# Future-Power-Networks/MAPDN

Measured on AMD Instinct MI355X. Metric: env-steps/sec (whole node), case141 batch=4096, at 1/2/4/8 MI355X, higher is better.
Workload: dtype f64

## Files before the change

include/mapdn.h:

```cpp
#ifndef MAPDN_H
#define MAPDN_H

#include <stdint.h>

#ifdef __cplusplus
extern "C" {
#endif

#define MAPDN_OK 0
#define MAPDN_E_INVALID (-1)
#define MAPDN_E_TOPOLOGY (-2)
#define MAPDN_E_HIP (-3)
#define MAPDN_E_STATE (-4)
#define MAPDN_E_NOMEM (-5)
#define MAPDN_E_INTERNAL (-6)

#define MAPDN_N_INFO 11

enum { MAPDN_BARRIER_L1 = 0, MAPDN_BARRIER_L2 = 1, MAPDN_BARRIER_COURANT_BELTRAMI = 2,
       MAPDN_BARRIER_BOWL = 3, MAPDN_BARRIER_BUMP = 4 };

enum { MAPDN_SS_PV = 1, MAPDN_SS_DEMAND = 2, MAPDN_SS_REACTIVE = 4, MAPDN_SS_VM_PU = 8,
       MAPDN_SS_VA_DEGREE = 16, MAPDN_SS_ALL = 31 };

// ... 75 lines not shown
} mapdn_env_config;

typedef struct mapdn_dims_t {
  int32_t n_envs, n_bus, n_line, n_load, n_sgen, n_agents, n_actions, obs_size, state_size, n_info;
  int32_t is_radial;
  int32_t max_zone_size;
} mapdn_dims_t;

typedef struct mapdn_handle mapdn_handle;

const char* mapdn_last_error(const mapdn_handle* h);

int mapdn_create(const mapdn_netspec* net, const mapdn_env_config* cfg, int32_t n_envs,
                 int32_t device, mapdn_handle** out);
void mapdn_destroy(mapdn_handle* h);
int mapdn_dims(const mapdn_handle* h, mapdn_dims_t* out);

int mapdn_set_profiles(mapdn_handle* h, const double* pv, const double* load_p, const double* load_q,
                       int64_t n_rows, int32_t time_delta_min, int32_t days);

int mapdn_get_profile_stats(const mapdn_handle* h, double* stdv, double* smax);

int mapdn_reset(mapdn_handle* h, const int64_t* start_rows, int32_t add_noise, int32_t max_tries,
                void* stream);

int mapdn_step(mapdn_handle* h, const void* actions, int32_t actions_dtype, int32_t add_noise,
               double* reward, uint8_t* terminated, double* info, void* stream);

int mapdn_step_obs(mapdn_handle* h, const void* actions, int32_t actions_dtype, int32_t add_noise,
                   double* reward, uint8_t* terminated, double* info, void* obs, int32_t obs_dtype, void* stream);

int mapdn_get_obs(mapdn_handle* h, void* obs, int32_t dtype, void* stream);
int mapdn_get_state(mapdn_handle* h, void* state, int32_t dtype, void* stream);

int mapdn_get_results(mapdn_handle* h, double* vm_pu, double* va_degree, double* p_mw, double* q_mvar,
                      double* pl_mw, double* sgen_p, double* sgen_q, void* stream);
int mapdn_get_loads(mapdn_handle* h, double* load_p, double* load_q, void* stream);

int mapdn_get_start_rows(mapdn_handle* h, int64_t* start_rows, void* stream);

int mapdn_get_auto_reset_mask(mapdn_handle* h, uint8_t* mask, void* stream);

int mapdn_get_returns(mapdn_handle* h, double* returns, void* stream);

int mapdn_solve_only(mapdn_handle* h, const double* p_load, const double* q_load, const double* p_sgen,
                     const double* q_sgen, double* vm_pu, double* va_degree, int32_t* iterations,
                     uint8_t* converged, void* stream);

int mapdn_get_ybus_dense(const mapdn_handle* h, double* ybus_re_im);
int mapdn_get_obs_index(const mapdn_handle* h, int32_t* kind, int32_t* index);

int mapdn_get_schedule(const mapdn_handle* h, int32_t n_waves, int32_t* n_rows, int32_t* rows, int32_t* parent);

int mapdn_get_nr_geometry(const mapdn_handle* h, int32_t* out20);

int mapdn_get_flat_factors(const mapdn_handle* h, double* factors, int32_t* bus_of_pos);

int mapdn_get_sparse_program(const mapdn_handle* h, int32_t sub_lanes, int32_t* dims, int32_t* ops, int32_t* order, int32_t* slots_ij);

int mapdn_dense_solve(const double* a, const double* b, double* x, int32_t n, int32_t batch, void* stream);

int mapdn_policy_forward(const float* obs, const float* hid_in, const float* w1, const float* b1, const float* ln_g,
                         const float* ln_b, const float* w_ih, const float* w_hh, const float* b_ih, const float* b_hh,
                         const float* w2, const float* b2, float* means, float* hid_out, int32_t rows, int32_t n_agents,
                         int32_t obs_dim, int32_t id_dim, float ln_eps, void* stream);

int mapdn_policy_forward_train(const float* obs, const float* hid_in, const float* w1, const float* b1, const float* ln_g,
                               const float* ln_b, const float* w_ih, const float* w_hh, const float* b_ih, const float* b_hh,
                               const float* w2, const float* b2, float* means, float* hid_out, float* x1_out, int32_t rows,
                               int32_t n_agents, int32_t obs_dim, int32_t id_dim, float ln_eps, void* stream);
int64_t mapdn_policy_backward_scratch_floats(int64_t rows);
int mapdn_policy_backward(const float* dmeans, const float* x1, const float* hid_in, const float* ln_g, const float* ln_b, float ln_eps,
                          const float* w_ih, const float* w_hh, const float* b_ih, const float* b_hh, const float* w2, float* dx1,
                          float* dgates, float* xn, float* small, float* scratch, int64_t rows, void* stream);

int mapdn_policy_forward_fits(int32_t obs_dim, int32_t id_dim);

int mapdn_layernorm64_forward(const float* x, const float* gamma, const float* beta, float* y, float* mean, float* rstd,
                              int64_t rows, float eps, int32_t relu, void* stream);
int mapdn_layernorm64_backward_blocks(int64_t rows);
int mapdn_layernorm64_backward(const float* dy, const float* x, const float* gamma, const float* beta, const float* mean,
                               const float* rstd, float* dx, float* dgamma, float* dbeta, float* partial, int64_t rows,
                               int32_t relu, void* stream);
int mapdn_layernorm64_bc_forward(const float* base, const float* per_n, int32_t n, const float* gamma, const float* beta, float* y,
                                 float* mean, float* rstd, int64_t rows, float eps, int32_t relu, void* stream);
int mapdn_layernorm64_bc_backward(const float* dy, const float* base, const float* per_n, int32_t n, const float* gamma, const float* beta,
                                  const float* mean, const float* rstd, float* dx, float* dgamma, float* dbeta, float* partial,
                                  int64_t rows, int32_t relu, void* stream);
int mapdn_relu_dot64_forward(const float* pre, const float* w, float bias, float* v, int64_t rows, void* stream);
int mapdn_relu_dot64_backward(const float* dv, const float* pre, const float* w, float* dpre, float* dw, float* db, float* partial,
                              int64_t rows, void* stream);

int mapdn_critic_head_forward(const float* x, const float* per_n, int32_t n, const float* gamma, const float* beta, float eps,
                              const float* w2, const float* b2, const float* w3, const float* b3, float* v, int64_t rows, void* stream);
int64_t mapdn_critic_head_scratch_floats(int64_t rows, int32_t n, int32_t formed);
int mapdn_critic_head_backward(const float* dv, const float* x, const float* per_n, int32_t n, const float* gamma, const float* beta,
                               float eps, const float* w2, const float* b2, const float* w3, const float* b3, float* dx, float* grads,
                               float* scratch, int64_t rows, int32_t param_grads, void* stream);
int mapdn_critic_head_mse(const float* ret, const float* wrow, const float* scale, const float* x, const float* per_n, int32_t n,
                          const float* gamma, const float* beta, float eps, const float* w2, const float* b2, const float* w3,
                          const float* b3, float* dx, float* grads, float* scratch, int64_t rows, void* stream);
int mapdn_critic_head_backward_dot(const float* dv, const float* x, const float* per_n, int32_t n, const float* gamma, const float* beta,
                                   float eps, const float* w2, const float* b2, const float* w3, const float* b3, const float* dot_w,
                                   float* dact, int64_t rows, void* stream);

int mapdn_explore_actions(const float* mean, const float* eps, const float* avail, float stdv, int32_t tanh_bound, double action_scale,
// ... 20 lines not shown
```

mapdn_amd/_lib.py:

```python
from __future__ import annotations

import ctypes as C
import os

import numpy as np

from .netspec import NetSpec

_HERE = os.path.dirname(os.path.abspath(__file__))
LIB_PATH = os.path.join(_HERE, "libmapdn_hip.so")

N_INFO = 11
INFO_KEYS = (
    "percentage_of_v_out_of_control", "percentage_of_lower_than_lower_v",
    "percentage_of_higher_than_upper_v", "totally_controllable_ratio",
    "average_voltage_deviation", "average_voltage", "max_voltage_drop_deviation",
    "max_voltage_rise_deviation", "total_line_loss", "q_loss", "destroy",
)
BARRIER_IDS = dict(l1=0, l2=1, courant_beltrami=2, bowl=3, bump=4)
SS_BITS = dict(pv=1, demand=2, reactive=4, vm_pu=8, va_degree=16)
F32, F64 = 0, 1

EXPORTS = (
    "mapdn_last_error", "mapdn_create", "mapdn_destroy", "mapdn_dims", "mapdn_set_profiles", "mapdn_reset",
    "mapdn_step", "mapdn_get_start_rows", "mapdn_get_returns", "mapdn_get_obs", "mapdn_get_state", "mapdn_get_results", "mapdn_get_loads",
    "mapdn_solve_only", "mapdn_get_ybus_dense", "mapdn_get_obs_index", "mapdn_get_schedule", "mapdn_get_flat_factors", "mapdn_stats", "mapdn_nr_timing",
    "mapdn_nr_time_ms", "mapdn_get_auto_reset_mask", "mapdn_dense_solve", "mapdn_step_obs", "mapdn_get_sparse_program", "mapdn_policy_forward",
    "mapdn_policy_forward_fits", "mapdn_layernorm64_forward", "mapdn_layernorm64_backward", "mapdn_layernorm64_backward_blocks",
    "mapdn_get_nr_geometry", "mapdn_debug_stream", "mapdn_build_info", "mapdn_layernorm64_bc_forward", "mapdn_layernorm64_bc_backward", "mapdn_relu_dot64_forward", "mapdn_relu_dot64_backward",
    "mapdn_critic_head_forward", "mapdn_critic_head_scratch_floats", "mapdn_critic_head_backward", "mapdn_critic_head_backward_dot", "mapdn_critic_head_mse", "mapdn_get_profile_stats",
    "mapdn_explore_actions", "mapdn_rollout_stats", "mapdn_copy_segments",
    "mapdn_policy_forward_train", "mapdn_policy_backward", "mapdn_policy_backward_scratch_floats",
)

_pd = C.POINTER(C.c_double)
_pi = C.POINTER(C.c_int32)
_pu8 = C.POINTER(C.c_uint8)


class CNetSpec(C.Structure):
    _fields_ = [
        ("n_bus", C.c_int32), ("bus_vn_kv", _pd), ("bus_zone", _pi),
        ("n_line", C.c_int32), ("line_from_bus", _pi), ("line_to_bus", _pi),
        ("line_r_ohm_per_km", _pd), ("line_x_ohm_per_km", _pd), ("line_c_nf_per_km", _pd),
        ("line_g_us_per_km", _pd), ("line_length_km", _pd), ("line_parallel", _pi), ("line_in_service", _pu8),
        ("n_branch_pu", C.c_int32), ("br_from_bus", _pi), ("br_to_bus", _pi), ("br_r_pu", _pd), ("br_x_pu", _pd),
        ("br_b_pu", _pd), ("br_ratio", _pd), ("br_shift_deg", _pd),
        ("n_shunt", C.c_int32), ("shunt_bus", _pi), ("shunt_p_mw", _pd), ("shunt_q_mvar", _pd),
        ("n_load", C.c_int32), ("load_bus", _pi),
        ("n_sgen", C.c_int32), ("sgen_bus", _pi), ("sgen_zone", _pi),
        ("ext_grid_bus", C.c_int32), ("ext_grid_vm_pu", C.c_double), ("sn_mva", C.c_double), ("f_hz", C.c_double),
        ("br_g_pu", _pd), ("load_scaling", _pd), ("sgen_scaling", _pd), ("bus_alias", _pi),
    ]


class CEnvConfig(C.Structure):
    _fields_ = [
        ("barrier_type", C.c_int32), ("voltage_weight", C.c_double), ("q_weight", C.c_double),
        ("line_weight", C.c_double), ("use_line_weight", C.c_int32), ("use_q_weight", C.c_int32),
        ("v_lower", C.c_double), ("v_upper", C.c_double), ("episode_limit", C.c_int32),
        ("action_low", C.c_double), ("action_high", C.c_double), ("reset_action", C.c_int32),
        ("state_space", C.c_int32), ("seed", C.c_uint64), ("env_id_offset", C.c_int64), ("auto_reset", C.c_int32),
        ("nr_solver", C.c_int32), ("nr_waves", C.c_int32), ("nr_lanes", C.c_int32), ("nr_lean", C.c_int32),
        ("nr_h_lds", C.c_int32), ("nr_g_lds", C.c_int32), ("nr_rec_lds", C.c_int32), ("nr_flat_lds", C.c_int32), ("nr_line_lds", C.c_int32),
        ("nr_mm_pass", C.c_int32), ("sp_lanes", C.c_int32), ("inject_full", C.c_int32),
        ("nr_check_dx", C.c_double), ("nr_check_quad", C.c_double), ("debug_geometry", C.c_int32),
        ("tolerance_mva", C.c_double), ("tolerance_is_pu", C.c_int32), ("nr_init", C.c_int32),
        ("fuse_inject", C.c_int32), ("overlap_advance", C.c_int32), ("xcd_map", C.c_int32),
    ]


TUNING_INT = ("nr_solver", "nr_waves", "nr_lanes", "nr_lean", "nr_h_lds", "nr_g_lds", "nr_rec_lds", "nr_flat_lds", "nr_line_lds",
              "nr_mm_pass", "sp_lanes", "inject_full", "debug_geometry", "tolerance_is_pu", "nr_init", "fuse_inject", "overlap_advance", "xcd_map")
TUNING_F64 = ("nr_check_dx", "nr_check_quad", "tolerance_mva")
NR_SOLVERS = dict(auto=0, tree=0, sparse=1, dense=2)
GEOMETRY_KEYS = ("solver", "waves", "lanes", "lean", "rows", "h_lds", "g_lds", "rec_lds", "flat_lds", "line_lds", "mm_pass",
                 "lds_bytes", "workgroups", "resident_per_cu", "rounds", "model_ns", "fuse_inject", "n_fused_buses", "n_nodes", "reserved")


class CDims(C.Structure):
    _fields_ = [(k, C.c_int32) for k in (
        "n_envs", "n_bus", "n_line", "n_load", "n_sgen", "n_agents", "n_actions", "obs_size", "state_size",
        "n_info", "is_radial", "max_zone_size")]


# ... 17 lines not shown
    global _lib
    if _lib is not None:
        return _lib
    import torch
    if "MAPDN_LIB_PATH" not in os.environ:
        from . import build as _build
        try:
            is_stale = _build.stale()
        except OSError:
            is_stale = not os.path.exists(LIB_PATH)
            if not is_stale:
                import warnings
                warnings.warn(f"mapdn_amd/csrc is not readable: {LIB_PATH} is loaded without the source-hash check", RuntimeWarning, stacklevel=2)
        if is_stale:
            try:
                _build.build_locked()
            except Exception as exc:
                raise ImportError(
                    f"{LIB_PATH} is missing or was built from other sources than mapdn_amd/csrc (hash {_build.library_hash()} vs "
                    f"{_safe_source_hash(_build)}) and could not be rebuilt ({exc}); build it with `python -m mapdn_amd.build` "
                    "(hipcc --offload-arch=gfx950); there is no CPU fallback") from exc
    lib = C.CDLL(os.environ.get("MAPDN_LIB_PATH", LIB_PATH))
    if "MAPDN_LIB_PATH" in os.environ:
        for name in EXPORTS:
            if not hasattr(lib, name):
                def _missing(*a, _n=name, **k):
                    raise AttributeError(f"{os.environ['MAPDN_LIB_PATH']} does not export {_n}")
                lib.__dict__[name] = _missing
    vp = C.c_void_p
    lib.mapdn_last_error.restype = C.c_char_p
    lib.mapdn_last_error.argtypes = [vp]
    lib.mapdn_build_info.restype = C.c_char_p
    lib.mapdn_build_info.argtypes = []
    lib.mapdn_create.argtypes = [C.POINTER(CNetSpec), C.POINTER(CEnvConfig), C.c_int32, C.c_int32, C.POINTER(vp)]
    lib.mapdn_destroy.argtypes = [vp]
    lib.mapdn_destroy.restype = None
    lib.mapdn_dims.argtypes = [vp, C.POINTER(CDims)]
    lib.mapdn_set_profiles.argtypes = [vp, _pd, _pd, _pd, C.c_int64, C.c_int32, C.c_int32]
    lib.mapdn_get_profile_stats.argtypes = [vp, _pd, _pd]
    lib.mapdn_reset.argtypes = [vp, vp, C.c_int32, C.c_int32, vp]
    lib.mapdn_step.argtypes = [vp, vp, C.c_int32, C.c_int32, vp, vp, vp, vp]
    lib.mapdn_step_obs.argtypes = [vp, vp, C.c_int32, C.c_int32, vp, vp, vp, vp, C.c_int32, vp]
    lib.mapdn_get_start_rows.argtypes = [vp, vp, vp]
    lib.mapdn_get_returns.argtypes = [vp, vp, vp]
    lib.mapdn_get_auto_reset_mask.argtypes = [vp, vp, vp]
    lib.mapdn_get_obs.argtypes = [vp, vp, C.c_int32, vp]
    lib.mapdn_get_state.argtypes = [vp, vp, C.c_int32, vp]
    lib.mapdn_get_results.argtypes = [vp] + [vp] * 7 + [vp]
    lib.mapdn_get_loads.argtypes = [vp, vp, vp, vp]
    lib.mapdn_solve_only.argtypes = [vp] + [vp] * 8 + [vp]
    lib.mapdn_get_ybus_dense.argtypes = [vp, _pd]
    lib.mapdn_get_obs_index.argtypes = [vp, _pi, _pi]
    lib.mapdn_get_schedule.argtypes = [vp, C.c_int32, _pi, _pi, _pi]
    lib.mapdn_get_flat_factors.argtypes = [vp, _pd, _pi]
    lib.mapdn_get_nr_geometry.argtypes = [vp, _pi]
    lib.mapdn_debug_stream.argtypes = [vp, vp, C.c_int32, C.c_int32, C.c_int32, vp]
    lib.mapdn_get_sparse_program.argtypes = [vp, C.c_int32, _pi, _pi, _pi, _pi]
    lib.mapdn_policy_forward.argtypes = [vp] * 14 + [C.c_int32] * 4 + [C.c_float, vp]
    lib.mapdn_policy_forward_fits.argtypes = [C.c_int32, C.c_int32]
    lib.mapdn_policy_forward_train.argtypes = [vp] * 15 + [C.c_int32] * 4 + [C.c_float, vp]
    lib.mapdn_policy_backward_scratch_floats.argtypes = [C.c_int64]
    lib.mapdn_policy_backward_scratch_floats.restype = C.c_int64
    lib.mapdn_policy_backward.argtypes = [vp] * 5 + [C.c_float] + [vp] * 10 + [C.c_int64, vp]
    lib.mapdn_layernorm64_forward.argtypes = [vp] * 6 + [C.c_int64, C.c_float, C.c_int32, vp]
    lib.mapdn_layernorm64_backward_blocks.argtypes = [C.c_int64]
    lib.mapdn_layernorm64_backward.argtypes = [vp] * 10 + [C.c_int64, C.c_int32, vp]
    lib.mapdn_layernorm64_bc_forward.argtypes = [vp, vp, C.c_int32] + [vp] * 5 + [C.c_int64, C.c_float, C.c_int32, vp]
    lib.mapdn_layernorm64_bc_backward.argtypes = [vp, vp, vp, C.c_int32] + [vp] * 8 + [C.c_int64, C.c_int32, vp]
    lib.mapdn_relu_dot64_forward.argtypes = [vp, vp, C.c_float, vp, C.c_int64, vp]
    lib.mapdn_relu_dot64_backward.argtypes = [vp] * 7 + [C.c_int64, vp]
    lib.mapdn_critic_head_forward.argtypes = [vp, vp, C.c_int32, vp, vp, C.c_float] + [vp] * 5 + [C.c_int64, vp]
    lib.mapdn_critic_head_scratch_floats.argtypes = [C.c_int64, C.c_int32, C.c_int32]
    lib.mapdn_critic_head_scratch_floats.restype = C.c_int64
    lib.mapdn_critic_head_backward.argtypes = [vp, vp, vp, C.c_int32, vp, vp, C.c_float] + [vp] * 7 + [C.c_int64, C.c_int32, vp]
    lib.mapdn_explore_actions.argtypes = [vp, vp, vp, C.c_float, C.c_int32, C.c_double, C.c_double, vp, vp, vp, C.c_int64, vp]
    lib.mapdn_rollout_stats.argtypes = [vp, vp, vp, vp, vp, vp, C.c_int32, vp]
    lib.mapdn_copy_segments.argtypes = [C.POINTER(vp), C.POINTER(vp), C.POINTER(C.c_int64), C.c_int32, vp]
    lib.mapdn_critic_head_mse.argtypes = [vp] * 5 + [C.c_int32, vp, vp, C.c_float] + [vp] * 7 + [C.c_int64, vp]
    lib.mapdn_critic_head_backward_dot.argtypes = [vp, vp, vp, C.c_int32, vp, vp, C.c_float] + [vp] * 6 + [C.c_int64, vp]
    lib.mapdn_dense_solve.argtypes = [vp, vp, vp, C.c_int32, C.c_int32, vp]
    lib.mapdn_stats.argtypes = [vp, C.POINTER(C.c_int64), C.POINTER(C.c_double), C.POINTER(C.c_int32), vp]
    lib.mapdn_nr_timing.argtypes = [vp, C.c_int32]
    lib.mapdn_nr_time_ms.argtypes = [vp, C.POINTER(C.c_double), C.POINTER(C.c_int64)]
    for name in EXPORTS:
        if name not in ("mapdn_last_error", "mapdn_destroy", "mapdn_build_info"):
            getattr(lib, name).restype = C.c_int
    _lib = lib
    return lib


def check(rc, handle=None):
    if rc != 0:
        msg = load().mapdn_last_error(handle)
        raise MapdnError(rc, msg.decode() if msg else "?")


def _p(a, typ):
    return a.ctypes.data_as(typ) if a.size else C.cast(None, typ)


def make_cnetspec(net: NetSpec):
    keep = net
    s = CNetSpec()
    s.n_bus = net.n_bus
    s.bus_vn_kv = _p(net.bus_vn_kv, _pd)
    s.bus_zone = _p(net.bus_zone, _pi)
# ... 78 lines not shown
```

mapdn_amd/csrc/capi.hip:

```cpp
#include <hip/hip_runtime.h>

#include <algorithm>
#include <cmath>
#include <cstdio>
#include <cstdlib>
#include <cstring>
#include <string>
#include <vector>

#include "kernels.hpp"
#include "colstats.hpp"
#include "plan.hpp"

using namespace mapdn;

struct mapdn_handle {
  Plan plan;
  Schedule sched;
  SparseProg sprog;
  int solver = 0;
  int sp_lanes = 0;
  mapdn_env_config cfg;
  Dev d;
  int device = 0;
// ... 797 lines not shown

int mapdn_get_ybus_dense(const mapdn_handle* h, double* out) try {
  if (!h || !out) return MAPDN_E_INVALID;
  const Plan& P = h->plan;
  for (size_t i = 0; i < P.ybus.size(); ++i) { out[2 * i] = P.ybus[i].real(); out[2 * i + 1] = P.ybus[i].imag(); }
  return MAPDN_OK;
} MAPDN_CATCH(h)

int mapdn_get_obs_index(const mapdn_handle* h, int32_t* kind, int32_t* index) try {
  if (!h || !kind || !index) return MAPDN_E_INVALID;
  std::memcpy(kind, h->plan.obs_kind.data(), h->plan.obs_kind.size() * sizeof(int32_t));
  std::memcpy(index, h->plan.obs_idx.data(), h->plan.obs_idx.size() * sizeof(int32_t));
  return MAPDN_OK;
} MAPDN_CATCH(h)

int mapdn_get_nr_geometry(const mapdn_handle* h, int32_t* out) try {
  if (!h || !out) return MAPDN_E_INVALID;
  const mapdn_handle::Geo& g = h->geo;
  const bool fuse_possible = h->solver == 0 && !h->cfg.auto_reset && !knob_int(h->cfg.inject_full, "MAPDN_INJECT_FULL") &&
                             knob_tri(h->cfg.fuse_inject, "MAPDN_FUSE_INJECT") != 2;
  const int32_t v[20] = {h->solver, g.W, g.L, g.lean, g.rows, g.h_lds, g.g_lds, g.rec_lds, g.flat_lds, g.line_lds, g.mm_pass,
                         (int32_t)h->lds_bytes, (int32_t)g.wgs, g.resident, g.rounds, (int32_t)std::min(g.model_ns, 2.0e9),
                         (h->host_only ? fuse_possible : h->fuse_inject) ? 1 : 0, (int32_t)h->plan.fused_obus.size(), h->plan.nb, 0};
  std::memcpy(out, v, sizeof(v));
  if (h->solver == 1) out[2] = h->sp_lanes;
  return MAPDN_OK;
} MAPDN_CATCH(h)

int mapdn_get_flat_factors(const mapdn_handle* h, double* factors, int32_t* bus_of_pos) try {
  if (!h || !factors) return MAPDN_E_INVALID;
  if (!h->plan.radial) return MAPDN_E_TOPOLOGY;
  Schedule S;
  build_schedule(h->plan, 1, S);
  const int n = h->plan.n;
  for (int r = 0; r < S.R; ++r) {
    const StepRec& T = S.steps[(size_t)r];
    if (T.flags & S_LIVE) std::memcpy(factors + (size_t)(T.kp & 0xffffu) * FLAT_N, &S.flat[(size_t)r * FLAT_N], FLAT_N * sizeof(double));
  }
  if (bus_of_pos) std::memcpy(bus_of_pos, h->plan.bus_of_pos.data(), (size_t)(n + 1) * sizeof(int32_t));
  return MAPDN_OK;
} MAPDN_CATCH(h)

int mapdn_get_schedule(const mapdn_handle* h, int32_t W, int32_t* n_rows, int32_t* rows, int32_t* parent) try {
  if (!h || !n_rows || W < 1 || W > 16) return MAPDN_E_INVALID;
  if (!h->plan.radial) return MAPDN_E_TOPOLOGY;
  Schedule S;
  build_schedule(h->plan, W, S);
  *n_rows = S.R;
  if (rows) for (size_t i = 0; i < S.steps.size(); ++i) rows[i] = (S.steps[i].flags & S_LIVE) ? (int32_t)(S.steps[i].kp & 0xffffu) : -1;
  if (parent) std::memcpy(parent, h->plan.par.data(), h->plan.par.size() * sizeof(int32_t));
  return MAPDN_OK;
} MAPDN_CATCH(h)

int mapdn_get_sparse_program(const mapdn_handle* h, int32_t S, int32_t* dims, int32_t* ops, int32_t* order, int32_t* slots_ij) try {
  if (!h || !dims || S < 1 || S > 64) return MAPDN_E_INVALID;
  SparseProg G;
  sparse_program(h->plan, S, G);
  dims[0] = G.n_blocks; dims[1] = G.n_fill; dims[2] = G.n_phases; dims[3] = G.rows_per_sub; dims[4] = G.max_nnz;
  dims[5] = (int32_t)(G.slots_ij.size() / 3);
  if (ops) std::memcpy(ops, G.ops.data(), G.ops.size() * sizeof(SpOp));
  if (order) std::memcpy(order, G.order.data(), G.order.size() * sizeof(int32_t));
  if (slots_ij) std::memcpy(slots_ij, G.slots_ij.data(), G.slots_ij.size() * sizeof(int32_t));
  return MAPDN_OK;
} MAPDN_CATCH(h)

int mapdn_dense_solve(const double* a, const double* b, double* x, int32_t n, int32_t batch, void* stream) try {
  if (!a || !b || !x) return MAPDN_E_INVALID;
  const int rc = dense_solve_debug(a, b, x, n, batch, (hipStream_t)stream);
  return rc == 0 ? MAPDN_OK : (rc == -1 ? MAPDN_E_INVALID : MAPDN_E_HIP);
} MAPDN_CATCH(nullptr)

int mapdn_stats(mapdn_handle* h, int64_t* reset_failures, double* mean_iters, int32_t* max_iters, void* stream) try {
  if (!h) return MAPDN_E_INVALID;
  NEEDDEV(h);
  HIPCHK(h, hipSetDevice(h->device));
  hipStream_t st = (hipStream_t)stream;
  launch_stats(h->d, h->stats_dev, st);
  long long host[4];
  HIPCHK(h, hipMemcpyAsync(host, h->stats_dev, sizeof(host), hipMemcpyDeviceToHost, st));
  HIPCHK(h, hipStreamSynchronize(st));
  if (reset_failures) *reset_failures = host[0];
  if (mean_iters) *mean_iters = host[2] ? (double)host[1] / (double)host[2] : 0.0;
  if (max_iters) *max_iters = (int32_t)host[3];
  return MAPDN_OK;
} MAPDN_CATCH(h)

int mapdn_nr_timing(mapdn_handle* h, int32_t enable) try {
  if (!h) return MAPDN_E_INVALID;
  h->timing = enable != 0;
  return MAPDN_OK;
} MAPDN_CATCH(h)

int mapdn_nr_time_ms(mapdn_handle* h, double* total_ms, int64_t* launches) try {
  if (!h) return MAPDN_E_INVALID;
  NEEDDEV(h);
  HIPCHK(h, hipSetDevice(h->device));
  double ms = h->acc_ms; int64_t n = h->acc_launches;
  for (size_t i = 0; i + 1 < h->ev_used; i += 2) {
    HIPCHK(h, hipEventSynchronize(h->ev[i + 1]));
    float t = 0.f;
    HIPCHK(h, hipEventElapsedTime(&t, h->ev[i], h->ev[i + 1]));
    ms += t; n += 1;
  }
  h->ev_used = 0; h->acc_ms = 0.0; h->acc_launches = 0;
  if (total_ms) *total_ms = ms;
  if (launches) *launches = n;
// ... 5 lines not shown
```

mapdn_amd/csrc/nr_tree.hpp:

```cpp
#pragma once
#include <hip/hip_runtime.h>
#include <stdint.h>

#include <type_traits>

#include "kernels.hpp"
#include "nr_common.hpp"

namespace mapdn {


#ifdef MAPDN_NR_STAMPS
static __device__ unsigned long long g_stamps[4096];
#define STAMP(id) do { if (stamp_on && ns < 4095) g_stamps[++ns] = ((unsigned long long)(id) << 48) | (__builtin_readcyclecounter() & 0xffffffffffffull); } while (0)
#ifdef MAPDN_NR_STAMPS_FINE
#define STAMP2(id) STAMP(id)
#else
#define STAMP2(id) do { } while (0)
#endif
#else
#define STAMP(id) do { } while (0)
#define STAMP2(id) do { } while (0)
#endif

// ... 491 lines not shown
            if (nch > 2) {
              auto gather = [&](unsigned slot) { const d2 a = cs[((size_t)slot * 4 + 3) * L]; aR0 += a.x; aR1 += a.y; };
              gather((chs >> 20) & 1023u);
              const unsigned cptr = clist_ptr(fl, slots, chs);
#pragma unroll 1
              for (int j = 3; j < nch; ++j) gather((unsigned)s_clist[cptr + j - 3]);
            }
          }
        }
        const double r0 = Fp - aR0, r1 = Fq - aR1;
        const double h0 = i0 * r0 + i1 * r1, h1 = i2 * r0 + i3 * r1;
        const double t0 = ap_i * h0 + ap_r * h1, t1 = ap_i * h1 - ap_r * h0;
        cR0 = t0; cR1 = t1;
        if (flu & SU_W_ANY) cs[((size_t)(slots & 1023u) * 4 + 3) * L] = d2{t0, t1};
        SCHED_FENCE();
        const unsigned k = kp & 0xffffu;
        if (HL) sH[(size_t)k * L] = d2{h0, h1}; else bst2(d2{h0, h1}, rs, voE + k * bb, sF_H);
        STAMP2(232);
        if (W > 1) lds_barrier();
        STAMP(102);
        ++r;
      }
    }
  };
  double dxm = 0.0;
  auto apply_update = [&](double y0, double y1, d2 vk, unsigned k, bool live) {
    dxm = fmax(dxm, live ? fmax(fabs(y0), fabs(y1)) : 0.0);
    double s, c;
    const double dth = -y0;
    sincos_small(dth, &s, &c);
    if (__any(live && !(fabs(dth) <= 0.5))) sincos_mid(dth, &s, &c);
    sV[(size_t)k * L] = done ? vk : nr_rotate(vk, s, c, y1);
  };
  constexpr int UPN = NR_UPDATE_GROUP;
  auto apply_update3 = [&](const d2 (&xx)[UPN], const d2 (&vv)[UPN], const unsigned (&kk)[UPN], const bool (&lv)[UPN]) {
    double s[UPN], c[UPN];
    bool big = false;
#pragma unroll
    for (int i = 0; i < UPN; ++i) {
      dxm = fmax(dxm, lv[i] ? fmax(fabs(xx[i].x), fabs(xx[i].y)) : 0.0);
      sincos_small(-xx[i].x, &s[i], &c[i]);
      big = big | (lv[i] & !(fabs(xx[i].x) <= 0.5));
    }
    if (__any(big)) {
#pragma unroll
      for (int i = 0; i < UPN; ++i) if (__any(lv[i] && !(fabs(xx[i].x) <= 0.5))) sincos_mid(-xx[i].x, &s[i], &c[i]);
    }
#pragma unroll
    for (int i = 0; i < UPN; ++i) sV[(size_t)kk[i] * L] = done ? vv[i] : nr_rotate(vv[i], s[i], c[i], xx[i].y);
  };
  auto bwd_xprop = [&](auto src) {
    constexpr int SRC = decltype(src)::value;
    constexpr bool gG = (SRC == 1) && !GL;
    u32x4 ixq[4]; d2 g01q[4], g23q[4];
    auto load_g = [&](int row, const u32x4& ixr, int slot) {
      if constexpr (SRC == 0) {
        if (flatL) { const char* p = flatT + (unsigned)row * FB; g01q[slot] = *(const d2*)(p + FL_G0 * 8); g23q[slot] = *(const d2*)(p + FL_G2 * 8); }
        else { const unsigned sf = row_s(row, FB); g01q[slot] = bld2(rsF, voF + FL_G0 * 8u, sf); g23q[slot] = bld2(rsF, voF + FL_G2 * 8u, sf); }
      } else if constexpr (gG) {
        const unsigned voN = voE + (ixr.w & 0xffffu) * bb;
        g01q[slot] = bld2(rs, voN, sF_G01); g23q[slot] = bld2(rs, voN, sF_G23);
      }
    };
    constexpr int KP = gG ? KR : 0;
    u32x4 ixs[KP > 0 ? KP : 1];
    static_for<KP>([&](auto ic) { constexpr int i = decltype(ic)::value; ixs[i] = load_ix(i); });
    ixq[0] = load_ix(R - 1); ixq[1] = load_ix(max(R - 2, 0)); ixq[2] = load_ix(max(R - 3, 0));
    load_g(R - 1, ixq[0], 0); load_g(max(R - 2, 0), ixq[1], 1);
    int r = R - 1;
    while (r >= KP) {
#pragma unroll
      for (int u = 0; u < 4; ++u) {
        if (r < KP) break;
        const uint32_t fl = ixq[u % 4].x, kp = ixq[u % 4].w;
        const unsigned k = kp & 0xffffu, p = kp >> 16;
        const d2 q = sH[(size_t)p * L];
        const d2 hh = sH[(size_t)k * L];
        d2 g01, g23;
        if constexpr (SRC == 1 && GL) { g01 = sG[(size_t)(2 * k) * L]; g23 = sG[(size_t)(2 * k + 1) * L]; }
        ixq[(u + 3) % 4] = load_ix(max(r - 3, KP));
        load_g(max(r - 2, KP), ixq[(u + 2) % 4], (u + 2) % 4);
        SCHED_FENCE();
        STAMP2(240);
        if constexpr (SRC == 0 || gG) { g01 = g01q[u % 4]; g23 = g23q[u % 4]; }
        const bool cout = (fl & S_CARRY_OUT) != 0;
        const double p0 = cout ? x0 : q.x, p1 = cout ? x1 : q.y;
        const double y0 = hh.x - (g01.x * p0 + g01.y * p1);
        const double y1 = hh.y - (g23.x * p0 + g23.y * p1);
        x0 = y0; x1 = y1;
        sH[(size_t)k * L] = d2{y0, y1};
        STAMP2(242);
        if (W > 1) lds_barrier();
        STAMP(110 + SRC);
        --r;
      }
    }
    static_for_down<KP>([&](auto ic) {
      constexpr int i = decltype(ic)::value;
      {
        const uint32_t fl = ixs[i].x, kp = ixs[i].w;
        const unsigned k = kp & 0xffffu, p = kp >> 16;
        const d2 q = sH[(size_t)p * L];
        const d2 hh = sH[(size_t)k * L];
        SCHED_FENCE();
        const bool cout = (fl & S_CARRY_OUT) != 0;
        const double p0 = cout ? x0 : q.x, p1 = cout ? x1 : q.y;
        const double G0 = a_get(Ga[i][0], Ga[i][1]), G1 = a_get(Ga[i][2], Ga[i][3]), G2 = a_get(Ga[i][4], Ga[i][5]), G3 = a_get(Ga[i][6], Ga[i][7]);
        const double y0 = hh.x - (G0 * p0 + G1 * p1);
        const double y1 = hh.y - (G2 * p0 + G3 * p1);
        x0 = y0; x1 = y1;
        sH[(size_t)k * L] = d2{y0, y1};
        if (W > 1) lds_barrier();
        STAMP(110 + SRC);
      }
    });
    for (unsigned kb = t; kb < n; kb += (unsigned)UPN * Wt) {
      unsigned kk[UPN]; d2 xx[UPN], vv[UPN]; bool lv[UPN];
#pragma unroll
      for (int i = 0; i < UPN; ++i) {
        const unsigned kx = kb + (unsigned)i * Wt;
        lv[i] = kx < n; kk[i] = lv[i] ? kx : n + 1u;
        xx[i] = sH[(size_t)kk[i] * L]; vv[i] = sV[(size_t)kk[i] * L];
      }
      apply_update3(xx, vv, kk, lv);
      STAMP(30);
    }
  };
  auto mismatch_pass = [&]() {
    const __amdgpu_buffer_rsrc_t rsP = __builtin_amdgcn_make_buffer_rsrc(const_cast<StepRec*>(d.mm_recs), 0, d.mm_recs_bytes, 0x00020000);
    const int NPs = d.mm_np;
    const unsigned voP = t * (unsigned)NPs * TB;
    {
      u32x4 ixn = bldu4(rsP, voP, 0u); d2 ypn = bld2(rsP, voP + 48u, 0u);
      for (int j = 0; j < NPs; ++j) {
        const u32x4 ix = ixn; const d2 ypk = ypn;
        const unsigned sn = row_s(min(j + 1, NPs - 1), TB);
        ixn = bldu4(rsP, voP, sn); ypn = bld2(rsP, voP + 48u, sn);
        const unsigned k = ix.w & 0xffffu, pp = ix.w >> 16;
        const d2 vk = sV[(size_t)k * L], vp = sV[(size_t)pp * L];
        const double ek = vk.x, fk = vk.y, ep = vp.x, fp = vp.y, gpk = ypk.x, bpk = ypk.y;
        const double ur = gpk * ek - bpk * fk, ui = gpk * fk + bpk * ek;
        const double apk_r = ep * ur + fp * ui, apk_i = fp * ur - ep * ui;
        sH[(size_t)k * L] = d2{apk_r, apk_i};
      }
    }
    STAMP(31);
    if (W > 1) lds_barrier();
    {
      const unsigned voSb = d.sb_off + e * 16u;
      auto cl = [&](int j) { return row_s(min(j, NPs - 1), TB); };
      u32x4 ixA = bldu4(rsP, voP, 0u), ixB = bldu4(rsP, voP, cl(1));
      d2 ykkN = bld2(rsP, voP + 16u, 0u), ykpN = bld2(rsP, voP + 32u, 0u), cksN = bld2(rsP, voP + 64u, 0u);
      d2 sbN = bld2(rs, voSb + (ixA.w & 0xffffu) * pb, 0u);
      for (int j = 0; j < NPs; ++j) {
        const u32x4 ix = ixA;
        const d2 ykk = ykkN, ykp = ykpN, cks = cksN, sb = sbN;
        const unsigned k = ix.w & 0xffffu, pp = ix.w >> 16;
        const int nch = (int)((ix.x >> 8) & 255u);
        const d2 vk = sV[(size_t)k * L], vp = sV[(size_t)pp * L];
        const d2 a0 = sH[(size_t)(ix.y & 0xffffu) * L], a1 = sH[(size_t)(ix.y >> 16) * L], a2 = sH[(size_t)(ix.z & 0xffffu) * L];
        {
          const unsigned s1 = cl(j + 1);
          ykkN = bld2(rsP, voP + 16u, s1); ykpN = bld2(rsP, voP + 32u, s1); cksN = bld2(rsP, voP + 64u, s1);
          sbN = bld2(rs, voSb + (ixB.w & 0xffffu) * pb, 0u);
          ixA = ixB; ixB = bldu4(rsP, voP, cl(j + 2));
        }
        const double gkk = ykk.x, bkk = ykk.y, gkp = ykp.x, bkp = ykp.y;
        const double ek = vk.x, fk = vk.y, ep = vp.x, fp = vp.y;
// ... 168 lines not shown
```

mapdn_amd/csrc/plan.cpp:

```cpp
#include "plan.hpp"

#include <algorithm>
#include <cmath>
#include <map>

namespace mapdn {

namespace {

struct PiBranch {
  int32_t f, t;
  cplx yff, yft, ytf, ytt;
};

PiBranch pi_from_line(const mapdn_netspec& net, int l) {
  const int f = net.line_from_bus[l], t = net.line_to_bus[l];
  const double vn = net.bus_vn_kv[f];
  const double base_r = vn * vn / net.sn_mva;
  const double len = net.line_length_km[l];
  const double par = (double)net.line_parallel[l];
  const double r = net.line_r_ohm_per_km[l] * len / base_r / par;
  const double x = net.line_x_ohm_per_km[l] * len / base_r / par;
  const double b = 2.0 * net.f_hz * M_PI * net.line_c_nf_per_km[l] * 1e-9 * base_r * len * par;
  const double g = net.line_g_us_per_km[l] * 1e-6 * base_r * len * par;
// ... 510 lines not shown
    }
    S.n_xslots = std::max(next, 1);
  }
  const uint32_t c_zero = (uint32_t)S.n_cslots, c_trash = c_zero + 1; S.n_cslots += 2;
  const uint32_t x_zero = (uint32_t)S.n_xslots, x_trash = x_zero + 1; S.n_xslots += 2;
  S.step_of_node.assign(n + 1, -1);
  for (int w = 0; w < W; ++w)
    for (int r = 0; r < R; ++r) {
      StepRec& T = S.steps[(size_t)w * R + r];
      const int k = rows[r][w];
      T = StepRec{};
      T.kp = (uint32_t)(n + 1) | ((uint32_t)n << 16);
      T.slots = c_trash | (x_trash << 10) | (x_zero << 20);
      T.chs = c_zero | (c_zero << 10) | (c_zero << 20);
      T.ykk[0] = 1.0; T.ykk[1] = -1.0; T.ykp[0] = -1.0; T.ykp[1] = 1.0; T.ypk[0] = -1.0; T.ypk[1] = 1.0;
      if (k < 0) continue;
      S.step_of_node[k] = w * R + r;
      const double* c = &P.yc[(size_t)k * 8];
      T.ykk[0] = c[0]; T.ykk[1] = c[1]; T.ykp[0] = c[2]; T.ykp[1] = c[3]; T.ypk[0] = c[4]; T.ypk[1] = c[5];
      T.cks[0] = c[6]; T.cks[1] = c[7];
      const int p = P.par[k];
      T.kp = (uint32_t)k | ((uint32_t)p << 16);
      uint32_t f = S_LIVE, os = c_trash, xsl = x_trash, pxs = x_zero;
      if (p == n) f |= S_PARENT_ROOT;
      else if (carry_out[k]) f |= S_CARRY_OUT;
      else { f |= S_SCRATCH_OUT; os = (uint32_t)oslot[k]; pxs = (uint32_t)xslot[p]; }
      std::vector<int> kids;
      const int cc = chain_child(k);
      if (cc >= 0) { if (carry_out[cc]) f |= S_CARRY_IN; else kids.push_back(oslot[cc]); }
      for (int ch : children[k]) if (ch != cc) kids.push_back(oslot[ch]);
      uint32_t ch3[3] = {c_zero, c_zero, c_zero};
      for (size_t j = 0; j < kids.size() && j < 3; ++j) ch3[j] = (uint32_t)kids[j];
      const uint32_t cptr = (uint32_t)S.clist.size();
      for (size_t j = 3; j < kids.size(); ++j) S.clist.push_back(kids[j]);
      if (xslot[k] >= 0) { f |= S_X_OUT; xsl = (uint32_t)xslot[k]; }
      T.slots = os | (xsl << 10) | (pxs << 20) | (((cptr >> 8) & 3u) << 30);
      T.chs = ch3[0] | (ch3[1] << 10) | (ch3[2] << 20) | (((cptr >> 10) & 3u) << 30);
      T.flags = f | ((uint32_t)std::min<size_t>(kids.size(), 255) << 16) | ((cptr & 255u) << 24);
    }
  for (int w0 = 0; w0 < W; w0 += Sw)
    for (int r = 0; r < R; ++r) {
      uint32_t gmax = 0, any = 0;
      for (int w = w0; w < w0 + Sw; ++w) {
        const StepRec& T = S.steps[(size_t)w * R + r];
        if (!(T.flags & S_LIVE)) continue;
        gmax = std::max(gmax, std::min<uint32_t>((T.flags >> 16) & 255u, 3u));
        if (T.flags & S_SCRATCH_OUT) any |= SU_W_ANY;
        if (T.flags & S_X_OUT) any |= SU_XW_ANY;
        if ((T.flags & S_SCRATCH_OUT)) any |= SU_XR_ANY;
        if (T.cks[0] != 0.0 || T.cks[1] != 0.0) any |= SU_SLACK_ANY;
      }
      for (int w = w0; w < w0 + Sw; ++w) S.steps[(size_t)w * R + r].flags |= (gmax << SU_GMAX_SHIFT) | any;
    }
  if (S.clist.empty()) S.clist.push_back(0);
  S.mm_ptr.assign(1, 0); S.mm_child.clear();
  for (int k = 0; k < n; ++k) {
    const int cc = chain_child(k);
    if (cc >= 0) S.mm_child.push_back(cc);
    for (int ch : children[k]) if (ch != cc) S.mm_child.push_back(ch);
    S.mm_ptr.push_back((int32_t)S.mm_child.size());
  }
  if (S.mm_child.empty()) S.mm_child.push_back(0);
  S.mm_np = (n + W - 1) / W;
  S.mm_recs.assign((size_t)W * S.mm_np, StepRec{});
  for (int w = 0; w < W; ++w)
    for (int j = 0; j < S.mm_np; ++j) {
      StepRec& T = S.mm_recs[(size_t)w * S.mm_np + j];
      const int kx = w + j * W;
      const bool live = kx < n;
      const int k = live ? kx : n - 1;
      const int c_lo = S.mm_ptr[k], nch = live ? S.mm_ptr[k + 1] - c_lo : 0;
      auto child = [&](int q) { return (uint32_t)(q < nch ? S.mm_child[c_lo + q] : n + 1); };
      T.flags = (live ? 1u : 0u) | ((uint32_t)std::min(nch, 255) << 8);
      T.slots = child(0) | (child(1) << 16);
      T.chs = child(2);
      T.kp = (uint32_t)k | ((uint32_t)P.par[k] << 16);
      const double* c = &P.yc[(size_t)k * 8];
      T.ykk[0] = c[0]; T.ykk[1] = c[1]; T.ykp[0] = c[2]; T.ykp[1] = c[3]; T.ypk[0] = c[4]; T.ypk[1] = c[5]; T.cks[0] = c[6]; T.cks[1] = c[7];
    }
  {
    const double v = P.vroot, v2 = v * v;
    std::vector<double> aS((size_t)n * 2, 0.0), aD((size_t)n * 4, 0.0), node((size_t)n * FLAT_N, 0.0);
    for (int k = 0; k < n; ++k) {
      const double* c = &P.yc[(size_t)k * 8];
      const double gkk = c[0], bkk = c[1], gkp = c[2], bkp = c[3], gpk = c[4], bpk = c[5];
      const double akp_r = v2 * gkp, akp_i = -v2 * bkp, apk_r = v2 * gpk, apk_i = -v2 * bpk;
      const double akk_r = v2 * gkk, akk_i = -v2 * bkk, aks_r = v * c[6], aks_i = -v * c[7];
      const double sr = (akk_r + aks_r) + akp_r + aS[2 * k], si = (akk_i + aks_i) + akp_i + aS[2 * k + 1];
      const double D0 = -(si - akk_i) - aD[4 * k], D1 = (sr + akk_r) - aD[4 * k + 1];
      const double D2 = (sr - akk_r) - aD[4 * k + 2], D3 = (si + akk_i) - aD[4 * k + 3];
      const double idet = 1.0 / (D0 * D3 - D1 * D2);
      const double I0 = D3 * idet, I1 = -D1 * idet, I2 = -D2 * idet, I3 = D0 * idet;
      const double G0 = I0 * akp_i - I1 * akp_r, G1 = I0 * akp_r + I1 * akp_i;
      const double G2 = I2 * akp_i - I3 * akp_r, G3 = I2 * akp_r + I3 * akp_i;
      double* o = &node[(size_t)k * FLAT_N];
      o[FL_SR] = sr; o[FL_SI] = si; o[FL_I0] = I0; o[FL_I1] = I1; o[FL_I2] = I2; o[FL_I3] = I3;
      o[FL_APR] = apk_r; o[FL_API] = apk_i; o[FL_G0] = G0; o[FL_G1] = G1; o[FL_G2] = G2; o[FL_G3] = G3;
      const int p = P.par[k];
      if (p < n) {
        aS[2 * p] += apk_r; aS[2 * p + 1] += apk_i;
        aD[4 * p] += apk_i * G0 + apk_r * G2; aD[4 * p + 1] += apk_i * G1 + apk_r * G3;
        aD[4 * p + 2] += apk_i * G2 - apk_r * G0; aD[4 * p + 3] += apk_i * G3 - apk_r * G1;
      }
    }
    S.flat.assign((size_t)W * R * FLAT_N, 0.0);
    for (int w = 0; w < W; ++w)
// ... 9 lines not shown
```

mapdn_amd/csrc/plan.hpp:

```cpp
#pragma once
#include <complex>
#include <cstdint>
#include <string>
#include <vector>

#include "../../include/mapdn.h"

namespace mapdn {

using cplx = std::complex<double>;

enum : uint32_t {
  F_PARENT_ROOT = 1u,
  F_PARENT_NEXT = 2u,
  F_CARRY_IN = 4u,
  F_SCRATCH_IN = 8u,
  F_SCRATCH_FIRST = 16u,
};

enum : int32_t {
  G_ZERO = 0, G_P_ADDBACK = 1, G_Q_ADDBACK = 2, G_SGEN_P = 3, G_SGEN_Q = 4, G_VM = 5, G_VA_RAD = 6,
  G_P = 7, G_Q = 8, G_VA_DEG = 9, G_NKIND = 10
};

struct StepRec {
  uint32_t flags, slots, chs, kp;
  double ykk[2], ykp[2], ypk[2];
  double cks[2];
};
static_assert(sizeof(StepRec) == 80, "StepRec must be 80 bytes (5 x dwordx4)");

enum : uint32_t {
  S_PARENT_ROOT = 1u,
  S_CARRY_OUT = 2u,
  S_CARRY_IN = 4u,
  S_SCRATCH_OUT = 8u,
  S_X_OUT = 16u,
  S_LIVE = 32u,
  SU_GMAX_SHIFT = 6u,
  SU_W_ANY = 256u,
  SU_XW_ANY = 512u,
  SU_XR_ANY = 1024u,
  SU_SLACK_ANY = 2048u,
};

struct Schedule {
  int32_t W = 1, R = 0;
  int32_t S = 1;
  std::vector<StepRec> steps;
  std::vector<int32_t> step_of_node;
  std::vector<int32_t> clist;
  int32_t n_cslots = 0, n_xslots = 0;
  std::vector<double> flat;
  std::vector<int32_t> mm_ptr, mm_child;
  int32_t mm_np = 0;
  std::vector<StepRec> mm_recs;
};
enum { FL_SR = 0, FL_SI, FL_I0, FL_I1, FL_I2, FL_I3, FL_APR, FL_API, FL_G0, FL_G1, FL_G2, FL_G3, FLAT_N };

struct LineFlow {
  int32_t fpos, tpos;
  double c[4];
};

struct Plan {
  int32_t nb = 0, n = 0;
  int32_t nl = 0, ns = 0, n_line = 0;
  int32_t root_bus = 0;
  double vroot = 1.0, sn_mva = 1.0, tol = 1e-8;
  bool radial = false;

  std::vector<int32_t> bus_of_pos, pos_of_bus;
  std::vector<int32_t> par;
  std::vector<uint32_t> flags;
  std::vector<double> yc;
  double yrr[2] = {0, 0};
  std::vector<int32_t> root_children;
  std::vector<double> root_y;
  std::vector<cplx> ybus;
  std::vector<int32_t> gy_ptr, gy_col;
  std::vector<double> gy_val;

  int32_t nbo = 0;
  std::vector<int32_t> pos_of_obus;
  std::vector<int32_t> cm_kind;
  std::vector<int32_t> fused_obus;
  std::vector<int32_t> ob_load_ptr, ob_load_idx, ob_sgen_ptr, ob_sgen_idx;
  std::vector<double> ob_shunt_p, ob_shunt_q;
  std::vector<int32_t> slack_group;
  std::vector<int32_t> alias_pos;

  std::vector<LineFlow> lines;
  std::vector<int32_t> load_ptr, load_idx, sgen_ptr, sgen_idx;
  std::vector<double> shunt_p, shunt_q;
  std::vector<int32_t> sgen_bus;
  std::vector<double> load_scale, sgen_scale;
// ... 39 lines not shown
```

Baseline: 39.38 million.

## Replace per-row LDS barriers in backward x-propagation with schedule-computed sparse barriers

The backward substitution in the tree NR solver used to issue an LDS barrier after every row when several waves cooperate. The schedule builder now marks only the rows where a cross-wave parent dependency requires synchronisation (SU_XBAR), and the kernel barriers only there, followed by a single barrier at the end. The kernel also prefetches the h values and G coefficients a few rows ahead to hide LDS latency. A debug export of the step words is added. Wrong barrier placement could cause races in the multi-wave case.

```diff
diff --git a/include/mapdn.h b/include/mapdn.h
--- a/include/mapdn.h
+++ b/include/mapdn.h
@@ -151,6 +151,8 @@
 
 int mapdn_get_schedule(const mapdn_handle* h, int32_t n_waves, int32_t* n_rows, int32_t* rows, int32_t* parent);
 
+int mapdn_get_nr_steps(const mapdn_handle* h, int32_t workers, int32_t per_wave, int32_t min_rows, int32_t* n_rows, uint32_t* words);
+
 int mapdn_get_nr_geometry(const mapdn_handle* h, int32_t* out20);
 
 int mapdn_get_flat_factors(const mapdn_handle* h, double* factors, int32_t* bus_of_pos);
diff --git a/mapdn_amd/_lib.py b/mapdn_amd/_lib.py
--- a/mapdn_amd/_lib.py
+++ b/mapdn_amd/_lib.py
@@ -30,7 +30,7 @@
     "mapdn_get_nr_geometry", "mapdn_debug_stream", "mapdn_build_info", "mapdn_layernorm64_bc_forward", "mapdn_layernorm64_bc_backward", "mapdn_relu_dot64_forward", "mapdn_relu_dot64_backward",
     "mapdn_critic_head_forward", "mapdn_critic_head_scratch_floats", "mapdn_critic_head_backward", "mapdn_critic_head_backward_dot", "mapdn_critic_head_mse", "mapdn_get_profile_stats",
     "mapdn_explore_actions", "mapdn_rollout_stats", "mapdn_copy_segments",
-    "mapdn_policy_forward_train", "mapdn_policy_backward", "mapdn_policy_backward_scratch_floats",
+    "mapdn_policy_forward_train", "mapdn_policy_backward", "mapdn_policy_backward_scratch_floats", "mapdn_get_nr_steps",
 )
 
 _pd = C.POINTER(C.c_double)
@@ -154,6 +154,7 @@
     lib.mapdn_get_ybus_dense.argtypes = [vp, _pd]
     lib.mapdn_get_obs_index.argtypes = [vp, _pi, _pi]
     lib.mapdn_get_schedule.argtypes = [vp, C.c_int32, _pi, _pi, _pi]
+    lib.mapdn_get_nr_steps.argtypes = [vp, C.c_int32, C.c_int32, C.c_int32, _pi, vp]
     lib.mapdn_get_flat_factors.argtypes = [vp, _pd, _pi]
     lib.mapdn_get_nr_geometry.argtypes = [vp, _pi]
     lib.mapdn_debug_stream.argtypes = [vp, vp, C.c_int32, C.c_int32, C.c_int32, vp]
diff --git a/mapdn_amd/csrc/capi.hip b/mapdn_amd/csrc/capi.hip
--- a/mapdn_amd/csrc/capi.hip
+++ b/mapdn_amd/csrc/capi.hip
@@ -873,6 +873,20 @@
   return MAPDN_OK;
 } MAPDN_CATCH(h)
 
+int mapdn_get_nr_steps(const mapdn_handle* h, int32_t workers, int32_t per_wave, int32_t min_rows, int32_t* n_rows, uint32_t* words) try {
+  if (!h || !n_rows || workers < 1 || per_wave < 1 || workers % per_wave || min_rows < 0) return MAPDN_E_INVALID;
+  if (!h->plan.radial) return MAPDN_E_TOPOLOGY;
+  Schedule S;
+  build_schedule(h->plan, workers, S, 0, per_wave, min_rows);
+  *n_rows = S.R;
+  if (words)
+    for (size_t i = 0; i < S.steps.size(); ++i) {
+      const StepRec& T = S.steps[i];
+      words[4 * i] = T.flags; words[4 * i + 1] = T.slots; words[4 * i + 2] = T.chs; words[4 * i + 3] = T.kp;
+    }
+  return MAPDN_OK;
+} MAPDN_CATCH(h)
+
 int mapdn_get_sparse_program(const mapdn_handle* h, int32_t S, int32_t* dims, int32_t* ops, int32_t* order, int32_t* slots_ij) try {
   if (!h || !dims || S < 1 || S > 64) return MAPDN_E_INVALID;
   SparseProg G;
diff --git a/mapdn_amd/csrc/nr_tree.hpp b/mapdn_amd/csrc/nr_tree.hpp
--- a/mapdn_amd/csrc/nr_tree.hpp
+++ b/mapdn_amd/csrc/nr_tree.hpp
@@ -567,7 +567,7 @@
   auto bwd_xprop = [&](auto src) {
     constexpr int SRC = decltype(src)::value;
     constexpr bool gG = (SRC == 1) && !GL;
-    u32x4 ixq[4]; d2 g01q[4], g23q[4];
+    u32x4 ixq[4]; d2 g01q[4], g23q[4], hq[4];
     auto load_g = [&](int row, const u32x4& ixr, int slot) {
       if constexpr (SRC == 0) {
         if (flatL) { const char* p = flatT + (unsigned)row * FB; g01q[slot] = *(const d2*)(p + FL_G0 * 8); g23q[slot] = *(const d2*)(p + FL_G2 * 8); }
@@ -575,37 +575,50 @@
       } else if constexpr (gG) {
         const unsigned voN = voE + (ixr.w & 0xffffu) * bb;
         g01q[slot] = bld2(rs, voN, sF_G01); g23q[slot] = bld2(rs, voN, sF_G23);
-      }
+      } else {
+        const unsigned kg = ixr.w & 0xffffu;
+        g01q[slot] = sG[(size_t)(2 * kg) * L]; g23q[slot] = sG[(size_t)(2 * kg + 1) * L];
+      }
+    };
+    auto parent_x = [&](uint32_t fl, unsigned p, double& p0, double& p1) {
+      d2 q = {0.0, 0.0};
+      if constexpr (W == 1) q = sH[(size_t)p * L];
+      else {
+        const uint32_t flu = uni(fl);
+        if (flu & SU_XBAR) lds_barrier();
+        if (flu & SU_XR_ANY) q = sH[(size_t)p * L];
+      }
+      const bool cout = (fl & S_CARRY_OUT) != 0;
+      p0 = cout ? x0 : q.x; p1 = cout ? x1 : q.y;
     };
     constexpr int KP = gG ? KR : 0;
     u32x4 ixs[KP > 0 ? KP : 1];
+    d2 hs[KP > 0 ? KP : 1];
     static_for<KP>([&](auto ic) { constexpr int i = decltype(ic)::value; ixs[i] = load_ix(i); });
-    ixq[0] = load_ix(R - 1); ixq[1] = load_ix(max(R - 2, 0)); ixq[2] = load_ix(max(R - 3, 0));
-    load_g(R - 1, ixq[0], 0); load_g(max(R - 2, 0), ixq[1], 1);
+    ixq[0] = load_ix(R - 1); ixq[1] = load_ix(max(R - 2, KP)); ixq[2] = load_ix(max(R - 3, KP));
+    load_g(R - 1, ixq[0], 0); load_g(max(R - 2, KP), ixq[1], 1);
+    hq[0] = sH[(size_t)(ixq[0].w & 0xffffu) * L];
+    static_for<KP>([&](auto ic) { constexpr int i = decltype(ic)::value; hs[i] = sH[(size_t)(ixs[i].w & 0xffffu) * L]; });
     int r = R - 1;
     while (r >= KP) {
 #pragma unroll
       for (int u = 0; u < 4; ++u) {
         if (r < KP) break;
         const uint32_t fl = ixq[u % 4].x, kp = ixq[u % 4].w;
-        const unsigned k = kp & 0xffffu, p = kp >> 16;
-        const d2 q = sH[(size_t)p * L];
-        const d2 hh = sH[(size_t)k * L];
-        d2 g01, g23;
-        if constexpr (SRC == 1 && GL) { g01 = sG[(size_t)(2 * k) * L]; g23 = sG[(size_t)(2 * k + 1) * L]; }
+        const unsigned k = kp & 0xffffu;
+        double p0, p1;
+        parent_x(fl, kp >> 16, p0, p1);
+        hq[(u + 1) % 4] = sH[(size_t)(ixq[(u + 1) % 4].w & 0xffffu) * L];
         ixq[(u + 3) % 4] = load_ix(max(r - 3, KP));
         load_g(max(r - 2, KP), ixq[(u + 2) % 4], (u + 2) % 4);
         SCHED_FENCE();
         STAMP2(240);
-        if constexpr (SRC == 0 || gG) { g01 = g01q[u % 4]; g23 = g23q[u % 4]; }
-        const bool cout = (fl & S_CARRY_OUT) != 0;
-        const double p0 = cout ? x0 : q.x, p1 = cout ? x1 : q.y;
+        const d2 hh = hq[u % 4], g01 = g01q[u % 4], g23 = g23q[u % 4];
         const double y0 = hh.x - (g01.x * p0 + g01.y * p1);
         const double y1 = hh.y - (g23.x * p0 + g23.y * p1);
         x0 = y0; x1 = y1;
         sH[(size_t)k * L] = d2{y0, y1};
         STAMP2(242);
-        if (W > 1) lds_barrier();
         STAMP(110 + SRC);
         --r;
       }
@@ -614,21 +627,20 @@
       constexpr int i = decltype(ic)::value;
       {
         const uint32_t fl = ixs[i].x, kp = ixs[i].w;
-        const unsigned k = kp & 0xffffu, p = kp >> 16;
-        const d2 q = sH[(size_t)p * L];
-        const d2 hh = sH[(size_t)k * L];
+        const unsigned k = kp & 0xffffu;
+        double p0, p1;
+        parent_x(fl, kp >> 16, p0, p1);
         SCHED_FENCE();
-        const bool cout = (fl & S_CARRY_OUT) != 0;
-        const double p0 = cout ? x0 : q.x, p1 = cout ? x1 : q.y;
+        const d2 hh = hs[i];
         const double G0 = a_get(Ga[i][0], Ga[i][1]), G1 = a_get(Ga[i][2], Ga[i][3]), G2 = a_get(Ga[i][4], Ga[i][5]), G3 = a_get(Ga[i][6], Ga[i][7]);
         const double y0 = hh.x - (G0 * p0 + G1 * p1);
         const double y1 = hh.y - (G2 * p0 + G3 * p1);
         x0 = y0; x1 = y1;
         sH[(size_t)k * L] = d2{y0, y1};
-        if (W > 1) lds_barrier();
         STAMP(110 + SRC);
       }
     });
+    if (W > 1) lds_barrier();
     for (unsigned kb = t; kb < n; kb += (unsigned)UPN * Wt) {
       unsigned kk[UPN]; d2 xx[UPN], vv[UPN]; bool lv[UPN];
 #pragma unroll
diff --git a/mapdn_amd/csrc/plan.cpp b/mapdn_amd/csrc/plan.cpp
--- a/mapdn_amd/csrc/plan.cpp
+++ b/mapdn_amd/csrc/plan.cpp
@@ -586,6 +586,22 @@
       }
       for (int w = w0; w < w0 + Sw; ++w) S.steps[(size_t)w * R + r].flags |= (gmax << SU_GMAX_SHIFT) | any;
     }
+  {
+    int last = R;
+    for (int r = R - 1; r >= 0; --r) {
+      bool need = false;
+      for (int w = 0; w < W; ++w) {
+        const int k = rows[r][w];
+        if (k < 0) continue;
+        const int p = P.par[k];
+        if (p == n || carry_out[k]) continue;
+        if (wave_of[p] / Sw != w / Sw && last >= row_of[p]) need = true;
+      }
+      if (!need) continue;
+      last = r;
+      for (int w = 0; w < W; ++w) S.steps[(size_t)w * R + r].flags |= SU_XBAR;
+    }
+  }
   if (S.clist.empty()) S.clist.push_back(0);
   S.mm_ptr.assign(1, 0); S.mm_child.clear();
   for (int k = 0; k < n; ++k) {
diff --git a/mapdn_amd/csrc/plan.hpp b/mapdn_amd/csrc/plan.hpp
--- a/mapdn_amd/csrc/plan.hpp
+++ b/mapdn_amd/csrc/plan.hpp
@@ -42,6 +42,7 @@
   SU_XW_ANY = 512u,
   SU_XR_ANY = 1024u,
   SU_SLACK_ANY = 2048u,
+  SU_XBAR = 4096u,
 };
 
 struct Schedule {
```

New measurement: 39.66 million, median of 6. No clear change (+0.7%).
